# minghanz/bev

Hardware: NVIDIA B200
Metric: BEV warp Mpix/s (higher is better)
Workload: dtype u8

## Files before the change

bev_b200/csrc/warp_fast.cu:

```cuda
#include "bevk_common.cuh"
#include "warp_u8c3.cuh"
#include "warp_f16c3.cuh"
#include "warp_formats.cuh"

#include <cuda.h>
#include <mutex>
#include <string.h>

namespace {

template <typename PX, bool LINEAR> constexpr int cta_threads()
{
    return LINEAR ? PX::kLinearThreads : PX::kNearestThreads;
}
__host__ __device__ constexpr int tile_w(int segs) { return 32 * segs; }
__host__ __device__ constexpr int tile_h(int segs, int warps) { return warps * (4 / segs); }
constexpr int kNarrowW = 12, kNarrowH = 16, kWideW = 4, kWideH = 8;
constexpr int kMapCount = kNarrowW * kNarrowH + kWideW * kWideH;
constexpr int kMaxBoxWidth = 2048, kMaxBoxHeight = 32;
constexpr int kMaxBoxes = 3;
constexpr int kMaxStageFrames = 8;
constexpr int kBarBytes = 256;
constexpr int kPrefetchAhead = 2;
constexpr int kTailSlack = 64;

__host__ __device__ constexpr int map_width(int wi)
{
    return wi < 8 ? 64 * (wi + 1) : (wi < 12 ? 512 + 128 * (wi - 7) : 1024 + 256 * (wi - 11));
}
__host__ __device__ constexpr bool map_is_wide(int wi) { return wi >= kNarrowW; }
__host__ __device__ constexpr int map_height(int hi)
{
    return hi < 8 ? hi + 1 : (hi < 12 ? 10 + 2 * (hi - 8) : 20 + 4 * (hi - 12));
}
__host__ __device__ __forceinline__ int map_width_index(int bytes)
{
    return bytes <= 512 ? (bytes + 63) / 64 - 1
                        : (bytes <= 1024 ? 7 + (bytes - 512 + 127) / 128 : 11 + (bytes - 1024 + 255) / 256);
}
__host__ __device__ __forceinline__ int map_height_index(int rows)
{
    return rows <= 8 ? rows - 1 : (rows <= 16 ? 8 + (rows - 9) / 2 : 12 + (rows - 17) / 4);
}
__host__ __device__ __forceinline__ int box_height(int wi, int rows)
{
    return map_is_wide(wi) ? (rows + 3) / 4 * 4 : map_height(map_height_index(rows));
}
__host__ __device__ __forceinline__ int box_map_index(int wi, int rows)
{
    return map_is_wide(wi) ? kNarrowW * kNarrowH + (wi - kNarrowW) * kWideH + (rows + 3) / 4 - 1
                           : wi * kNarrowH + map_height_index(rows);
}

struct WarpFastMaps {
    CUtensorMap m[kMapCount];
};

constexpr int kMaxChunks = 12;
struct ChunkPlan {
    int n_chunks;
    uint32_t cum[kMaxChunks + 1];
};

constexpr int kRecWords = 8;
constexpr int kHdrInts = 8;
struct WarpScratch {
    int *next_item;
    int *ready;
    int *hdr;
    uint32_t *rec;
    uint32_t recip_per_chunk, recip_tiles, recip_tiles_y;
};

__device__ __forceinline__ uint32_t smem_u32(const void *p)
{
    return (uint32_t)__cvta_generic_to_shared(p);
}
__device__ __forceinline__ void mbar_init(uint32_t bar, uint32_t count)
{
    asm volatile("mbarrier.init.shared::cta.b64 [%0], %1;" ::"r"(bar), "r"(count));
}
__device__ __forceinline__ void mbar_expect_tx(uint32_t bar, uint32_t bytes)
{
    asm volatile("mbarrier.arrive.expect_tx.shared::cta.b64 _, [%0], %1;" ::"r"(bar), "r"(bytes)
                 : "memory");
}
__device__ __forceinline__ void mbar_arrive(uint32_t bar)
{
    asm volatile("mbarrier.arrive.shared::cta.b64 _, [%0];" ::"r"(bar) : "memory");
}
__device__ __forceinline__ void mbar_wait(uint32_t bar, uint32_t parity)
{
    asm volatile(
        "{\n\t"
        ".reg .pred p;\n\t"
        "WAIT_%=:\n\t"
        "mbarrier.try_wait.parity.shared::cta.b64 p, [%0], %1;\n\t"
        "@p bra DONE_%=;\n\t"
        "bra WAIT_%=;\n\t"
        "DONE_%=:\n\t"
        "}" ::"r"(bar),
        "r"(parity)
        : "memory");
}
__device__ __forceinline__ void tma_box_g2s(uint32_t dst, const CUtensorMap *map, int x, int y,
                                            uint32_t bar)
{
    asm volatile(
        "cp.async.bulk.tensor.2d.shared::cluster.global.mbarrier::complete_tx::bytes"
        " [%0], [%1, {%3, %4}], [%2];" ::"r"(dst),
        "l"(reinterpret_cast<uint64_t>(map)), "r"(bar), "r"(x), "r"(y)
        : "memory");
}
__device__ __forceinline__ void tma_box_prefetch(const CUtensorMap *map, int x, int y)
{
    asm volatile("cp.async.bulk.prefetch.tensor.2d.L2.global [%0, {%1, %2}];" ::"l"(
                     reinterpret_cast<uint64_t>(map)),
                 "r"(x), "r"(y)
                 : "memory");
}
__device__ __forceinline__ uint32_t lds32(uint32_t addr)
{
    uint32_t v;
    asm volatile("ld.shared.u32 %0, [%1];" : "=r"(v) : "r"(addr));
    return v;
}
__device__ __forceinline__ int ld_acquire(const int *p)
{
    int v;
    asm volatile("ld.acquire.gpu.global.s32 %0, [%1];" : "=r"(v) : "l"(p) : "memory");
    return v;
}
__device__ __forceinline__ void st_release(int *p, int v)
{
    asm volatile("st.release.gpu.global.s32 [%0], %1;" ::"l"(p), "r"(v) : "memory");
}
__device__ __forceinline__ void keep(uint32_t &v) { asm volatile("" : "+r"(v)); }
__device__ __forceinline__ void keep(int &v) { asm volatile("" : "+r"(v)); }

struct BoxPlan {
    int n_boxes;
    int x;
    int y0;
    uint32_t bytes;
    int frame0, frame_step;
    int src_h;
    int n_frames, fps;
    int slog;
    uint32_t ring, full0;
    uint32_t stride, frame_bytes, pitch;
    int map_idx[kMaxBoxes];
    int row[kMaxBoxes];
};

struct ItemDesc {
    int item;
    int gi, tile_x, tile_y;
    int f0, n_frames;
    int first, stride;
    int chunk;
    int ready;
};

struct LoopCtx {
    uint32_t ring, full0;
    uint32_t stride;
    uint32_t frame_bytes;
    uint32_t pitch;
    int fps;
    int n_frames;
    int slog;
    int ahead;
    const WarpFastMaps *maps;
    const BoxPlan *plan;
};

template <bool TO_SMEM>
__device__ __noinline__ void produce(const BoxPlan *plan, const WarpFastMaps *maps, int i0,
                                     uint32_t use, int lane)
{
    const BoxPlan &pl = *plan;
    const int nf = min(pl.fps, pl.n_frames - i0);
    const int nb = pl.n_boxes;
    const int f = nb == 1 ? lane : (nb == 2 ? lane >> 1 : (lane * 11) >> 5);
    const int b = lane - f * nb;
    const bool mine = f < nf;
    const int row = pl.row[mine ? b : 0];
    const CUtensorMap *map = &maps->m[pl.map_idx[mine ? b : 0]];
    const int y = (pl.frame0 + (i0 + f) * pl.frame_step) * pl.src_h + pl.y0 + row;
    if (TO_SMEM) {
        const uint32_t slot = use & ((1u << pl.slog) - 1u);
        const uint32_t fb = pl.full0 + 8 * slot;
        mbar_wait(fb + (8u << pl.slog), ((use >> pl.slog) & 1u) ^ 1u);
        if (lane == 0) mbar_expect_tx(fb, pl.bytes * nf);
        __syncwarp();
        if (mine)
            tma_box_g2s(pl.ring + slot * pl.stride + f * pl.frame_bytes + row * pl.pitch, map, pl.x, y, fb);
    } else if (mine) {
        tma_box_prefetch(map, pl.x, y);
    }
}

template <int WARPS>
__device__ __forceinline__ void feed(const LoopCtx &c, int done, uint32_t use, int lane, int warp)
{
    const int turn = ((int)use - warp) & (WARPS - 1);
    const int i_load = done + (c.ahead - 1) * c.fps;
    if (turn == 0 && i_load < c.n_frames) produce<true>(c.plan, c.maps, i_load, use + c.ahead, lane);
    if (c.slog == 1 && turn == WARPS / 2 && i_load + kPrefetchAhead * c.fps < c.n_frames)
        produce<false>(c.plan, c.maps, i_load + kPrefetchAhead * c.fps, 0, lane);
}

template <int WARPS, typename BODY, typename STARTED>
__device__ __forceinline__ uint32_t stage_loop(const LoopCtx &c, uint32_t use, uint8_t *d,
                                               const uint32_t d_step, const int tid, BODY body, STARTED started)
{
    const uint32_t smask = (1u << c.slog) - 1u;
    const int lane = tid & 31, warp = tid >> 5;
    if (warp == 0) {
        for (int s = 0; s < c.ahead && s * c.fps < c.n_frames; ++s)
            produce<true>(c.plan, c.maps, s * c.fps, use + s, lane);
        for (int s = c.ahead; c.slog == 1 && s < c.ahead + kPrefetchAhead && s * c.fps < c.n_frames; ++s)
            produce<false>(c.plan, c.maps, s * c.fps, 0, lane);
        if (tid == 0) started();
    }
    int done = 0;
#pragma unroll 1
    while (done < c.n_frames) {
        const uint32_t slot = use & smask;
        const uint32_t fb = c.full0 + 8 * slot;
        mbar_wait(fb, (use >> c.slog) & 1u);
        uint32_t sa = c.ring + slot * c.stride;
        int nf = min(c.fps, c.n_frames - done);
        done += nf;
#pragma unroll 1
        for (; nf > 0; --nf, sa += c.frame_bytes, d += d_step) body(sa, d);
        __syncwarp();
        if (lane == 0) mbar_arrive(fb + (8u << c.slog));
        feed<WARPS>(c, done, use, lane, warp);
        ++use;
    }
    return use;
}

template <int SEGS, bool PAIRS> __device__ __forceinline__ int warp_px_x(int warp)
{
    if (!PAIRS) return 0;
    return SEGS >= 2 ? 64 * (warp % (SEGS >= 2 ? SEGS / 2 : 1)) : 0;
}
template <int SEGS, bool PAIRS> __device__ __forceinline__ int warp_px_y(int warp)
{
    if (!PAIRS) return warp * (4 / SEGS);
    return SEGS >= 2 ? 2 * (warp / (SEGS >= 2 ? SEGS / 2 : 1)) : 4 * warp;
}
template <int SEGS, bool PAIRS> __device__ __forceinline__ constexpr int px_seg(int k)
{
    return PAIRS ? (SEGS >= 2 ? (k >> 1) : 0) : k % SEGS;
}
template <int SEGS, bool PAIRS> __device__ __forceinline__ constexpr int px_row(int k)
{
    return PAIRS ? (SEGS >= 2 ? (k & 1) : k) : k / SEGS;
}

struct PairReg {
    uint32_t addr;
    uint32_t sh;
    uint32_t sel_f, sel_s;
    uint32_t sel_y;
    uint32_t wf0, wf1;
    uint32_t ws0, ws1;
};

// ... 22 lines not shown
{
    const uint32_t rnd = 32768u;
    {
        const uint32_t x0 = prmt(a0.g0, a0.g1, q.sel_f), x1 = prmt(a1.g0, a1.g1, q.sel_f);
        const uint32_t t0 = __dp2a_lo(q.wf1, x1, __dp2a_lo(q.wf0, x0, rnd));
        const uint32_t t1 = __dp2a_hi(q.wf1, x1, __dp2a_hi(q.wf0, x0, rnd));
        const uint32_t t2 = __dp2a_lo(q.wf1, ya1, __dp2a_lo(q.wf0, ya0, rnd));
        pf = prmt(prmt(t0, t1, 0x4462u), t2, 0x7610u);
    }
    {
        const uint32_t x0 = prmt(b0.g0, b0.g1, q.sel_s), x1 = prmt(b1.g0, b1.g1, q.sel_s);
        const uint32_t t0 = __dp2a_lo(q.ws1, x1, __dp2a_lo(q.ws0, x0, rnd));
        const uint32_t t1 = __dp2a_hi(q.ws1, x1, __dp2a_hi(q.ws0, x0, rnd));
        const uint32_t t2 = __dp2a_hi(q.ws1, yb1, __dp2a_hi(q.ws0, yb0, rnd));
        ps = prmt(prmt(t0, t1, 0x4462u), t2, 0x7610u);
    }
}

template <typename PX, bool LINEAR, int MINB, int SEGS>
__global__ void __launch_bounds__((cta_threads<PX, LINEAR>()), MINB)
warp_fast_kernel(const __grid_constant__ BevkWarpParams p,
                      const __grid_constant__ WarpFastMaps maps,
                      const __grid_constant__ ChunkPlan plan, const int tiles_x, const int tiles_y,
                      const int total_items, const int ring_bytes, const WarpScratch sc)
{
    constexpr int kThreads = cta_threads<PX, LINEAR>(), kWarps = kThreads / 32;
    extern __shared__ __align__(128) uint8_t smem[];
    uint64_t *bars = reinterpret_cast<uint64_t *>(smem + ring_bytes);
    __shared__ int s_box[4];
    __shared__ int s_any;
    __shared__ uint32_t s_use[3];
    __shared__ ItemDesc s_item[2];
    __shared__ double s_M[BEVK_MAX_GROUPS][9];
    __shared__ BoxPlan s_plan;

    const int tid = threadIdx.x, lane = tid & 31, warp = tid >> 5;
    const uint32_t ring = smem_u32(smem);
    const uint32_t bar0 = smem_u32(bars);
    if (tid == 0) {
        for (int sl = 1; sl <= 3; ++sl) {
            const int S = 1 << sl, base = 16 * S - 32;
            for (int i = 0; i < S; ++i) {
                mbar_init(bar0 + base + 8 * i, 1);
                mbar_init(bar0 + base + 8 * (S + i), kWarps);
            }
            s_use[sl - 1] = 0;
        }
        asm volatile("fence.mbarrier_init.release.cluster;" ::: "memory");
    }

    const int n_tiles = tiles_x * tiles_y;
    const uint8_t *src = (const uint8_t *)p.src;
    uint8_t *dst = (uint8_t *)p.dst;
    constexpr int kBpp = PX::kBpp;
    constexpr bool kPairMap = LINEAR && PX::kPairs;
    const int src_row_bytes = p.src_w * kBpp;
    const long long src_frame_bytes = (long long)src_row_bytes * p.src_h;
    const long long dst_frame_bytes = (long long)p.dst_w * p.dst_h * kBpp;

    const int per_chunk = p.n_groups * n_tiles;
    auto fast_div = [](int n, int d, uint32_t recip) {
        uint32_t q = __umulhi((uint32_t)n, recip);
        if (q * (uint32_t)d > (uint32_t)n) --q;
        if ((q + 1u) * (uint32_t)d <= (uint32_t)n) ++q;
        return (int)q;
    };
    auto decode = [&](int item, ItemDesc &o) {
        o.item = item;
        if (item >= total_items) return;
        const int chunk = fast_div(item, per_chunk, sc.recip_per_chunk), rem = item - chunk * per_chunk;
        const int gi = fast_div(rem, n_tiles, sc.recip_tiles), tile = rem - gi * n_tiles;
        o.gi = gi;
        o.tile_x = fast_div(tile, tiles_y, sc.recip_tiles_y);
        o.tile_y = tile - o.tile_x * tiles_y;
        const int count = p.g[gi].count;
        o.f0 = (int)(((unsigned long long)count * plan.cum[chunk]) >> 16);
        o.n_frames = (int)(((unsigned long long)count * plan.cum[chunk + 1]) >> 16) - o.f0;
        o.first = p.g[gi].first;
        o.stride = p.g[gi].stride;
        o.chunk = chunk;
        o.ready = (sc.ready != nullptr && chunk > 0)
                      ? ld_acquire(sc.ready + (gi * n_tiles + o.tile_x * tiles_y + o.tile_y))
                      : 1;
    };
    for (int i = tid; i < p.n_groups * 9; i += kThreads) s_M[i / 9][i % 9] = p.g[i / 9].M[i % 9];
    if (tid == 0) {
        decode(atomicAdd(sc.next_item, 1), s_item[0]);
        s_box[0] = s_box[2] = 1 << 30;
        s_box[1] = s_box[3] = -1;
        s_any = 0;
    }
    __syncthreads();
    const bool bw0_pow2 = (p.bw0 & (p.bw0 - 1)) == 0;
    const uint32_t row_bytes = (uint32_t)p.dst_w * (uint32_t)kBpp;

    int par = 0;
#pragma unroll 1
    while (true) {
        const int item = s_item[par].item;
        if (item >= total_items) break;
        const int gi = s_item[par].gi, tile_x = s_item[par].tile_x, tile_y = s_item[par].tile_y;
        const int f0 = s_item[par].f0, n_frames = s_item[par].n_frames;
        const int g_first = s_item[par].first, g_stride = s_item[par].stride;
        const int chunk = s_item[par].chunk;
        const bool published = s_item[par].ready != 0;
        int next_raw = 0;
        if (tid == 0) next_raw = atomicAdd(sc.next_item, 1);
        const int x0 = tile_x * tile_w(SEGS) + warp_px_x<SEGS, kPairMap>(warp);
        const int y0 = tile_y * tile_h(SEGS, kWarps) + warp_px_y<SEGS, kPairMap>(warp);
        const int tile_id = gi * n_tiles + tile_x * tiles_y + tile_y;
        par ^= 1;

        int cs[4], rs[4];
        uint32_t wpk[4];
        int bx0, bx1, by0, by1;
        bool any;
        if (sc.ready == nullptr || chunk == 0) {
            bx0 = by0 = 1 << 30;
            bx1 = by1 = -1;
#pragma unroll
            for (int k = 0; k < 4; ++k) {
                const int x = x0 + lane + 32 * px_seg<SEGS, kPairMap>(k), y = y0 + px_row<SEGS, kPairMap>(k);
                const bool in_dst = (x < p.dst_w) && (y < p.dst_h);
                int X, Y, wc0, wc1, wr0, wr1;
                const int xc = min(x, p.dst_w - 1);
                const int xb = bw0_pow2 ? (xc & ~(p.bw0 - 1)) : (xc / p.bw0) * p.bw0;
                bevk_map_pixel_xb(s_M[gi], xb, xc - xb, min(y, p.dst_h - 1), LINEAR ? 32.0 : 1.0, X, Y);
                if (LINEAR) {
                    const int sx = bevk_sat16(X >> 5), sy = bevk_sat16(Y >> 5);
// ... 44 lines not shown
                    int4 *h = reinterpret_cast<int4 *>(sc.hdr + (size_t)tile_id * kHdrInts);
                    __stcg(h, make_int4(bx0, bx1, by0, by1));
                    __stcg(h + 1, make_int4(any ? 1 : 0, 0, 0, 0));
                }
                __threadfence();
            }
        } else {
            if (!published) {
                if (tid == 0) {
                    const int *flag = sc.ready + tile_id;
                    while (ld_acquire(flag) == 0) __nanosleep(100);
                }
            }
            __syncthreads();
            const int4 *h = reinterpret_cast<const int4 *>(sc.hdr + (size_t)tile_id * kHdrInts);
            const int4 hb = __ldcg(h), hf = __ldcg(h + 1);
            bx0 = hb.x;
            bx1 = hb.y;
            by0 = hb.z;
            by1 = hb.w;
            any = hf.x != 0;
            const uint32_t *rec = sc.rec + (size_t)tile_id * (kRecWords * kThreads) + tid;
#pragma unroll
            for (int k = 0; k < 4; ++k) {
                const uint32_t pos = __ldcg(rec + (2 * k) * kThreads);
                cs[k] = (int)(pos & 0xffffu);
                rs[k] = (int)(pos >> 16);
                wpk[k] = __ldcg(rec + (2 * k + 1) * kThreads);
            }
        }

        const int a0 = (kBpp * bx0) & ~15;
        const int need_w = ((kBpp * (bx1 + 1) + 15) & ~15) - a0;
        const int wi = map_width_index(need_w);
        const int pitch = map_width(wi);
        const int nrows = by1 - by0 + 1;
        bool staged = any && need_w <= kMaxBoxWidth && nrows <= kMaxBoxes * kMaxBoxHeight;
        int box_rows = 0;
        if (staged)
            for (int rem = nrows; rem > 0;) {
                const int h = box_height(wi, min(rem, kMaxBoxHeight));
                box_rows += h;
                rem -= h;
            }
        const uint32_t frame_bytes = ((uint32_t)(box_rows * pitch) + 127u) & ~127u;
        staged = staged && 2 * frame_bytes <= (uint32_t)ring_bytes;
        if (!LINEAR && frame_bytes > 3u * 1024u * (uint32_t)kBpp) staged = false;
        const int fps = 4 * kMaxStageFrames * frame_bytes <= (uint32_t)ring_bytes ? kMaxStageFrames
                        : 4 * 4 * frame_bytes <= (uint32_t)ring_bytes ? 4
                        : 8 * frame_bytes <= (uint32_t)ring_bytes ? 2 : 1;
        const int stage_stride = fps * (int)frame_bytes;
        const int slog = (8 * stage_stride <= ring_bytes) ? 3 : (4 * stage_stride <= ring_bytes ? 2 : 1);
        const uint32_t full0 = bar0 + 16 * (1 << slog) - 32;
        if (tid == 0) {
            if (staged) {
                int rem = nrows, row = 0, nb = 0;
                while (rem > 0) {
                    const int r = min(rem, kMaxBoxHeight);
                    s_plan.map_idx[nb] = box_map_index(wi, r);
                    s_plan.row[nb] = row;
                    row += box_height(wi, r);
                    rem -= box_height(wi, r);
                    ++nb;
                }
                s_plan.n_boxes = nb;
                s_plan.x = map_is_wide(wi) ? a0 >> 3 : a0 >> 2;
                s_plan.y0 = by0;
                s_plan.bytes = (uint32_t)(box_rows * pitch);
                s_plan.frame0 = g_first + f0 * g_stride;
                s_plan.frame_step = g_stride;
                s_plan.src_h = p.src_h;
                s_plan.n_frames = n_frames;
                s_plan.fps = fps;
                s_plan.slog = slog;
                s_plan.ring = ring;
                s_plan.full0 = full0;
                s_plan.stride = stage_stride;
                s_plan.frame_bytes = frame_bytes;
                s_plan.pitch = pitch;
            }
        }
        __syncthreads();
        if (tid == 0) {
            if (sc.ready != nullptr && chunk == 0) st_release(sc.ready + tile_id, 1);
            s_box[0] = s_box[2] = 1 << 30;
            s_box[1] = s_box[3] = -1;
            s_any = 0;
        }
        auto next_item_decode = [&]() { decode(next_raw, s_item[par]); };

        const typename PX::Store st = PX::store_setup(lane);
        bool seg_ok[4];
#pragma unroll
        for (int k = 0; k < 4; ++k) {
            const int valid_px = min(32, p.dst_w - (x0 + 32 * px_seg<SEGS, kPairMap>(k)));
            seg_ok[k] = (y0 + px_row<SEGS, kPairMap>(k) < p.dst_h) && PX::lane_stores(lane, valid_px);
        }
        auto seg_ptr = [row_bytes](uint8_t *dd, uint8_t *dd1, int k) -> uint8_t * {
            const int row = px_row<SEGS, kPairMap>(k), seg = px_seg<SEGS, kPairMap>(k);
            return (row & 1 ? dd1 : dd) + (row >> 1) * 2 * (size_t)row_bytes + PX::kSegBytes * seg;
        };
        uint32_t d_step = (uint32_t)g_stride * (uint32_t)dst_frame_bytes;
        keep(d_step);
        uint8_t *d = dst + (long long)(g_first + f0 * g_stride) * dst_frame_bytes +
                     ((long long)y0 * p.dst_w + x0) * kBpp + PX::lane_offset(lane);

        if ((!any || !staged) && tid == 0) next_item_decode();
        if (!any) {
#pragma unroll 1
            for (int i = 0; i < n_frames; ++i, d += d_step)
#pragma unroll
                for (int k = 0; k < 4; ++k) PX::store_zero(seg_ptr(d, d + row_bytes, k), seg_ok[k], lane);
        } else if (staged) {
            LoopCtx c;
            c.ring = ring;
            c.full0 = full0;
            c.stride = stage_stride;
            c.frame_bytes = frame_bytes;
            c.pitch = pitch;
            c.fps = fps;
            c.n_frames = n_frames;
            c.slog = slog;
            c.ahead = slog == 1 ? 2 : (1 << slog) - 1;
            c.maps = &maps;
            c.plan = &s_plan;
            keep(c.ring);
            keep(c.full0);
            keep(c.slog);
            uint32_t use = s_use[slog - 1];

            int var = 3;
            if constexpr (LINEAR && PX::kPairs) {
                bool ok0 = true, ok1 = true, ok2 = true;
#pragma unroll
                for (int j = 0; j < 2; ++j) {
                    const int a = 2 * j, b = a + 1;
                    const bool aa = wpk[a] != 0, ab = wpk[b] != 0;
                    if (aa && ab) {
                        const int dr = rs[b] - rs[a], dc = cs[b] - cs[a];
                        const bool near = dc >= -1 && dc <= 1;
                        ok0 = ok0 && near && dr == 0;
                        ok1 = ok1 && near && dr == 1;
                        ok2 = ok2 && near && dr == -1;
                    } else if (aa || ab) {
                        const int r = aa ? rs[a] : rs[b];
                        ok1 = ok1 && (aa ? r + 2 <= by1 : r - 1 >= by0);
                        ok2 = ok2 && (ab ? r + 2 <= by1 : r - 1 >= by0);
                    } else {
                        ok1 = ok1 && by1 - by0 >= 2;
                        ok2 = ok2 && by1 - by0 >= 2;
                    }
                }
                var = __all_sync(0xffffffffu, ok0) ? 0
                      : (__all_sync(0xffffffffu, ok1) ? 1 : (__all_sync(0xffffffffu, ok2) ? 2 : 3));
            }
            if constexpr (LINEAR && PX::kPairs) if (var != 3) {
                PairReg pr[2];
                uint32_t ok = 0;
// ... 142 lines not shown
    long long rows = 0;
    unsigned long long stamp = 0;
    WarpFastMaps maps;
};
constexpr int kMapCacheSize = 8;
MapCacheEntry g_map_cache[kMapCacheSize];
unsigned long long g_map_stamp = 0;
std::mutex g_map_mutex;
EncodeTiledFn g_encode = nullptr;

int get_maps(const void *base, int row_bytes, long long rows, WarpFastMaps &out)
{
    std::lock_guard<std::mutex> lock(g_map_mutex);
    if (!g_encode) {
        void *fn = nullptr;
        cudaDriverEntryPointQueryResult qres;
        BEVK_CUDA(cudaGetDriverEntryPoint("cuTensorMapEncodeTiled", &fn, cudaEnableDefault, &qres));
        if (qres != cudaDriverEntryPointSuccess || !fn)
            BEVK_FAIL(BEVK_E_CUDA, "cuTensorMapEncodeTiled is not available from this driver");
        g_encode = (EncodeTiledFn)fn;
    }
    MapCacheEntry *victim = &g_map_cache[0];
    for (int i = 0; i < kMapCacheSize; ++i) {
        MapCacheEntry &e = g_map_cache[i];
        if (e.base == base && e.row_bytes == row_bytes && e.rows == rows) {
            e.stamp = ++g_map_stamp;
            out = e.maps;
            return BEVK_OK;
        }
        if (e.stamp < victim->stamp) victim = &e;
    }
    const cuuint64_t gstride[1] = {(cuuint64_t)row_bytes};
    const cuuint32_t estride[2] = {1, 1};
    for (int wi = 0; wi < kNarrowW + kWideW; ++wi) {
        const bool wide = map_is_wide(wi);
        const int es = wide ? 8 : 4;
        const cuuint64_t gdim[2] = {(cuuint64_t)(row_bytes / es), (cuuint64_t)rows};
        for (int hi = 0; hi < (wide ? kWideH : kNarrowH); ++hi) {
            const int h = wide ? 4 * (hi + 1) : map_height(hi);
            const cuuint32_t box[2] = {(cuuint32_t)(map_width(wi) / es), (cuuint32_t)h};
            CUresult r = g_encode(&victim->maps.m[box_map_index(wi, h)],
                                  wide ? CU_TENSOR_MAP_DATA_TYPE_UINT64 : CU_TENSOR_MAP_DATA_TYPE_UINT32,
                                  2, const_cast<void *>(base), gdim, gstride, box, estride,
                                  CU_TENSOR_MAP_INTERLEAVE_NONE, CU_TENSOR_MAP_SWIZZLE_NONE,
                                  CU_TENSOR_MAP_L2_PROMOTION_L2_128B,
                                  CU_TENSOR_MAP_FLOAT_OOB_FILL_NONE);
            if (r != CUDA_SUCCESS) {
                victim->base = nullptr;
                BEVK_FAIL(BEVK_E_CUDA, "cuTensorMapEncodeTiled failed (code %d) for a %ux%u box",
                          (int)r, box[0] * es, box[1]);
            }
        }
    }
    victim->base = base;
    victim->row_bytes = row_bytes;
    victim->rows = rows;
    victim->stamp = ++g_map_stamp;
    out = victim->maps;
    return BEVK_OK;
}

struct KernelConfig {
    bool ready = false;
    int ctas_per_sm = 0;
    int ring_bytes = 0;
};
template <typename PX, bool LINEAR> constexpr int min_ctas()
{
    return LINEAR ? PX::kLinearCtas : 4 * (256 / cta_threads<PX, LINEAR>());
}
constexpr int kMaxDevices = 64;
struct DeviceState {
    KernelConfig cfg[5][2][3];
    int sm_count = 0;
    bool pool_ready = false;
};
DeviceState g_dev[kMaxDevices];
inline int segs_index(int segs) { return segs == 4 ? 0 : (segs == 2 ? 1 : 2); }

inline int format_index(int dtype, int channels)
{
    if (dtype == BEVK_U8) return channels == 3 ? 0 : (channels == 1 ? 2 : (channels == 4 ? 3 : -1));
    if (dtype == BEVK_F16) return channels == 3 ? 1 : -1;
    if (dtype == BEVK_F32) return channels == 3 ? 4 : -1;
// ... 88 lines not shown
        for (int iy = 0; iy < nsy; ++iy)
            for (int ix = 0; ix < nsx; ++ix) {
                const int ty = nsy > 1 ? (int)((long long)iy * (tiles_y - 1) / (nsy - 1)) : 0;
                const int tx = nsx > 1 ? (int)((long long)ix * (tiles_x - 1) / (nsx - 1)) : 0;
                const int x0 = tx * tw, y0 = ty * th;
                const int x1 = (x0 + tw < p.dst_w ? x0 + tw : p.dst_w) - 1;
                const int y1 = (y0 + th < p.dst_h ? y0 + th : p.dst_h) - 1;
                const int cx[4] = {x0, x1, x0, x1}, cy[4] = {y0, y0, y1, y1};
                int lo_x = 1 << 30, hi_x = -(1 << 30), lo_y = 1 << 30, hi_y = -(1 << 30), pos = 0, neg = 0;
                for (int c = 0; c < 4; ++c) {
                    const double w = M[6] * cx[c] + M[7] * cy[c] + M[8];
                    pos += w > 0;
                    neg += w < 0;
                    int X, Y;
                    bevk_map_pixel(M, cx[c], cy[c], p.bw0, scale, X, Y);
                    const int sx = bevk_sat16(linear ? (X >> 5) : X), sy = bevk_sat16(linear ? (Y >> 5) : Y);
                    lo_x = sx < lo_x ? sx : lo_x;
                    hi_x = sx > hi_x ? sx : hi_x;
                    lo_y = sy < lo_y ? sy : lo_y;
                    hi_y = sy > hi_y ? sy : hi_y;
                }
                hi_x += linear;
                hi_y += linear;
                if (hi_x < 0 || hi_y < 0 || lo_x >= p.src_w || lo_y >= p.src_h) continue;
                if (pos != 4 && neg != 4) continue;
                ++active;
                lo_x = lo_x < 0 ? 0 : lo_x;
                lo_y = lo_y < 0 ? 0 : lo_y;
                hi_x = hi_x > p.src_w - 1 ? p.src_w - 1 : hi_x;
                hi_y = hi_y > p.src_h - 1 ? p.src_h - 1 : hi_y;
                const int a0 = (bpp * lo_x) & ~15;
                const int need_w = ((bpp * (hi_x + 1) + 15) & ~15) - a0 + 16;
                const int rows = hi_y - lo_y + 1 + 1;
                const int pitch = need_w <= kMaxBoxWidth ? map_width(map_width_index(need_w)) : need_w;
                if (need_w > kMaxBoxWidth || rows > kMaxBoxes * kMaxBoxHeight ||
                    2LL * pitch * (rows + 3) > ring_bytes)
                    ++bad;
            }
    }
    return active ? (double)bad / (double)active : 0.0;
}

struct ModeKey {
    double M[BEVK_MAX_GROUPS][9];
    int n_groups, src_h, src_w, dst_h, dst_w, linear, bpp, warps;
};
struct ModeEntry {
    ModeKey key;
    int segs;
    int best;
    bool split;
    unsigned long long stamp = 0;
    bool valid = false;
};
constexpr double kMaxSplit = 0.35;
constexpr int kModeCacheSize = 8;
ModeEntry g_mode_cache[kModeCacheSize];
unsigned long long g_mode_stamp = 0;

int pick_tile_shape(const BevkWarpParams &p, int linear, int bpp, int warps, int ring_bytes, bool force, bool *split)
{
    const double kNegligible = linear ? 0.002 : 0.05;
    ModeKey key;
    memset(&key, 0, sizeof(key));
    for (int i = 0; i < p.n_groups; ++i) memcpy(key.M[i], p.g[i].M, sizeof(key.M[i]));
    key.n_groups = p.n_groups;
    key.src_h = p.src_h;
    key.src_w = p.src_w;
    key.dst_h = p.dst_h;
// ... 108 lines not shown
    if (rc) return rc;

    const int tiles_x = (p.dst_w + tile_w(segs) - 1) / tile_w(segs);
    const int tiles_y = (p.dst_h + tile_h(segs, warps) - 1) / tile_h(segs, warps);
    const long long n_tiles = (long long)tiles_x * tiles_y;
    const int ctas = ds.sm_count * cfg.ctas_per_sm;

    ChunkPlan plan;
    memset(&plan, 0, sizeof(plan));
    const long long tile_groups = n_tiles * p.n_groups;
    if (max_count >= 128 && tile_groups * 5 >= 2LL * ctas) {
        static const uint32_t cum[8] = {0, 20480, 36864, 49152, 57344, 61952, 64512, 65536};
        plan.n_chunks = 7;
        memcpy(plan.cum, cum, sizeof(cum));
    } else {
        int k = (int)((3LL * ctas + tile_groups - 1) / tile_groups);
        k = k < 1 ? 1 : k;
        k = k > kMaxChunks ? kMaxChunks : k;
        k = k > (max_count + 7) / 8 ? (max_count + 7) / 8 : k;
        k = k < 1 ? 1 : k;
        plan.n_chunks = k;
        for (int i = 0; i <= k; ++i) plan.cum[i] = (uint32_t)(65536LL * i / k);
    }
    const long long items = tile_groups * plan.n_chunks;
    if (items > 0x7fffffffLL) return 0;
    const int grid = (int)(items < ctas ? items : ctas);

    const bool share_setup = (fmt == 0 || fmt == 2) && linear && plan.n_chunks > 1 &&
                             tile_groups * kRecWords * threads * 4 <= (512LL << 20);
    const size_t off_hard = 256;
    const size_t off_ready = off_hard + (((size_t)(split ? tile_groups : 0) + 255) & ~(size_t)255);
    const size_t off_hdr = off_ready + (((size_t)(share_setup ? tile_groups * 4 : 0) + 255) & ~(size_t)255);
    const size_t off_rec = off_hdr + (share_setup ? (size_t)tile_groups * kHdrInts * 4 : 0);
    const size_t total = off_rec + (share_setup ? (size_t)tile_groups * kRecWords * threads * 4 : 0);
    unsigned char *scratch = nullptr;
    BEVK_CUDA(cudaMallocAsync((void **)&scratch, total, stream));
    cudaError_t e = cudaMemsetAsync(scratch, 0, off_hdr, stream);
    WarpScratch sc;
    sc.next_item = (int *)scratch;
    sc.ready = share_setup ? (int *)(scratch + off_ready) : nullptr;
    sc.hdr = share_setup ? (int *)(scratch + off_hdr) : nullptr;
    sc.rec = share_setup ? (uint32_t *)(scratch + off_rec) : nullptr;
    auto recip = [](long long d) { return d <= 1 ? 0xffffffffu : (uint32_t)(((1ULL << 32) + d - 1) / d); };
    sc.recip_per_chunk = recip(tile_groups);
    sc.recip_tiles = recip(n_tiles);
    sc.recip_tiles_y = recip(tiles_y);
    if (split) {
        p.hard = scratch + off_hard;
        p.hard_tw = tile_w(segs);
        p.hard_th = tile_h(segs, warps);
        p.hard_ty = tiles_y;
        p.hard_tiles = (int)n_tiles;
    }

    int rc2 = 0;
    if (e == cudaSuccess) {
        const int smem = cfg.ring_bytes + kBarBytes + kTailSlack;
        with_format(fmt, [&](auto px) {
            launch_any<decltype(px)>(linear, segs, grid, smem, stream, p, maps, plan, tiles_x, tiles_y, (int)items,
                                     cfg.ring_bytes, sc);
            return 0;
        });
        e = cudaGetLastError();
        if (e == cudaSuccess && split) {
            rc2 = bevk_plan_generic_chunks(p, channels);
            if (!rc2) rc2 = bevk_launch_warp_generic(p, channels, dtype, linear, stream);
        }
    }
    const cudaError_t ef = cudaFreeAsync(scratch, stream);
    if (e != cudaSuccess) {
        bevk_set_error("staged warp launch failed: %s", cudaGetErrorString(e));
        return BEVK_E_CUDA;
    }
    if (rc2) return rc2;
    BEVK_CUDA(ef);
// ... 3 lines not shown
```

Baseline: 686,700.

## Build per-item TMA descriptors on device with exact box dims

```diff
diff --git a/bev_b200/csrc/warp_fast.cu b/bev_b200/csrc/warp_fast.cu
--- a/bev_b200/csrc/warp_fast.cu
+++ b/bev_b200/csrc/warp_fast.cu
@@ -15,45 +15,14 @@
 }
 __host__ __device__ constexpr int tile_w(int segs) { return 32 * segs; }
 __host__ __device__ constexpr int tile_h(int segs, int warps) { return warps * (4 / segs); }
-constexpr int kNarrowW = 12, kNarrowH = 16, kWideW = 4, kWideH = 8;
-constexpr int kMapCount = kNarrowW * kNarrowH + kWideW * kWideH;
-constexpr int kMaxBoxWidth = 2048, kMaxBoxHeight = 32;
-constexpr int kMaxBoxes = 3;
+constexpr int kMaxNarrowWidth = 1024, kMaxBoxWidth = 2048, kMaxBoxRows = 256;
 constexpr int kMaxStageFrames = 8;
 constexpr int kBarBytes = 256;
 constexpr int kPrefetchAhead = 2;
 constexpr int kTailSlack = 64;
 
-__host__ __device__ constexpr int map_width(int wi)
-{
-    return wi < 8 ? 64 * (wi + 1) : (wi < 12 ? 512 + 128 * (wi - 7) : 1024 + 256 * (wi - 11));
-}
-__host__ __device__ constexpr bool map_is_wide(int wi) { return wi >= kNarrowW; }
-__host__ __device__ constexpr int map_height(int hi)
-{
-    return hi < 8 ? hi + 1 : (hi < 12 ? 10 + 2 * (hi - 8) : 20 + 4 * (hi - 12));
-}
-__host__ __device__ __forceinline__ int map_width_index(int bytes)
-{
-    return bytes <= 512 ? (bytes + 63) / 64 - 1
-                        : (bytes <= 1024 ? 7 + (bytes - 512 + 127) / 128 : 11 + (bytes - 1024 + 255) / 256);
-}
-__host__ __device__ __forceinline__ int map_height_index(int rows)
-{
-    return rows <= 8 ? rows - 1 : (rows <= 16 ? 8 + (rows - 9) / 2 : 12 + (rows - 17) / 4);
-}
-__host__ __device__ __forceinline__ int box_height(int wi, int rows)
-{
-    return map_is_wide(wi) ? (rows + 3) / 4 * 4 : map_height(map_height_index(rows));
-}
-__host__ __device__ __forceinline__ int box_map_index(int wi, int rows)
-{
-    return map_is_wide(wi) ? kNarrowW * kNarrowH + (wi - kNarrowW) * kWideH + (rows + 3) / 4 - 1
-                           : wi * kNarrowH + map_height_index(rows);
-}
-
 struct WarpFastMaps {
-    CUtensorMap m[kMapCount];
+    CUtensorMap m[2];
 };
 
 constexpr int kMaxChunks = 12;
@@ -69,6 +38,7 @@
     int *ready;
     int *hdr;
     uint32_t *rec;
+    CUtensorMap *tmaps;
     uint32_t recip_per_chunk, recip_tiles, recip_tiles_y;
 };
 
@@ -119,6 +89,24 @@
                  "r"(x), "r"(y)
                  : "memory");
 }
+__device__ __forceinline__ void tmap_set_box_dim(uint32_t smap, int dim, int v)
+{
+    if (dim == 0)
+        asm volatile("tensormap.replace.tile.box_dim.shared::cta.b1024.b32 [%0], 0, %1;" ::"r"(smap), "r"(v) : "memory");
+    else
+        asm volatile("tensormap.replace.tile.box_dim.shared::cta.b1024.b32 [%0], 1, %1;" ::"r"(smap), "r"(v) : "memory");
+}
+__device__ __forceinline__ void tmap_publish(CUtensorMap *gmap, uint32_t smap)
+{
+    asm volatile("tensormap.cp_fenceproxy.global.shared::cta.tensormap::generic.release.gpu.sync.aligned"
+                 " [%0], [%1], 128;" ::"l"(reinterpret_cast<uint64_t>(gmap)), "r"(smap)
+                 : "memory");
+}
+__device__ __forceinline__ void tmap_acquire(const CUtensorMap *gmap)
+{
+    asm volatile("fence.proxy.tensormap::generic.acquire.gpu [%0], 128;" ::"l"(reinterpret_cast<uint64_t>(gmap))
+                 : "memory");
+}
 __device__ __forceinline__ uint32_t lds32(uint32_t addr)
 {
     uint32_t v;
@@ -139,7 +127,7 @@
 __device__ __forceinline__ void keep(int &v) { asm volatile("" : "+r"(v)); }
 
 struct BoxPlan {
-    int n_boxes;
+    const CUtensorMap *map;
     int x;
     int y0;
     uint32_t bytes;
@@ -148,9 +136,7 @@
     int n_frames, fps;
     int slog;
     uint32_t ring, full0;
-    uint32_t stride, frame_bytes, pitch;
-    int map_idx[kMaxBoxes];
-    int row[kMaxBoxes];
+    uint32_t stride, frame_bytes;
 };
 
 struct ItemDesc {
@@ -171,23 +157,16 @@
     int n_frames;
     int slog;
     int ahead;
-    const WarpFastMaps *maps;
     const BoxPlan *plan;
 };
 
 template <bool TO_SMEM>
-__device__ __noinline__ void produce(const BoxPlan *plan, const WarpFastMaps *maps, int i0,
-                                     uint32_t use, int lane)
+__device__ __noinline__ void produce(const BoxPlan *plan, int i0, uint32_t use, int lane)
 {
     const BoxPlan &pl = *plan;
     const int nf = min(pl.fps, pl.n_frames - i0);
-    const int nb = pl.n_boxes;
-    const int f = nb == 1 ? lane : (nb == 2 ? lane >> 1 : (lane * 11) >> 5);
-    const int b = lane - f * nb;
-    const bool mine = f < nf;
-    const int row = pl.row[mine ? b : 0];
-    const CUtensorMap *map = &maps->m[pl.map_idx[mine ? b : 0]];
-    const int y = (pl.frame0 + (i0 + f) * pl.frame_step) * pl.src_h + pl.y0 + row;
+    const bool mine = lane < nf;
+    const int y = (pl.frame0 + (i0 + lane) * pl.frame_step) * pl.src_h + pl.y0;
     if (TO_SMEM) {
         const uint32_t slot = use & ((1u << pl.slog) - 1u);
         const uint32_t fb = pl.full0 + 8 * slot;
@@ -195,9 +174,9 @@
         if (lane == 0) mbar_expect_tx(fb, pl.bytes * nf);
         __syncwarp();
         if (mine)
-            tma_box_g2s(pl.ring + slot * pl.stride + f * pl.frame_bytes + row * pl.pitch, map, pl.x, y, fb);
+            tma_box_g2s(pl.ring + slot * pl.stride + lane * pl.frame_bytes, pl.map, pl.x, y, fb);
     } else if (mine) {
-        tma_box_prefetch(map, pl.x, y);
+        tma_box_prefetch(pl.map, pl.x, y);
     }
 }
 
@@ -206,9 +185,9 @@
 {
     const int turn = ((int)use - warp) & (WARPS - 1);
     const int i_load = done + (c.ahead - 1) * c.fps;
-    if (turn == 0 && i_load < c.n_frames) produce<true>(c.plan, c.maps, i_load, use + c.ahead, lane);
+    if (turn == 0 && i_load < c.n_frames) produce<true>(c.plan, i_load, use + c.ahead, lane);
     if (c.slog == 1 && turn == WARPS / 2 && i_load + kPrefetchAhead * c.fps < c.n_frames)
-        produce<false>(c.plan, c.maps, i_load + kPrefetchAhead * c.fps, 0, lane);
+        produce<false>(c.plan, i_load + kPrefetchAhead * c.fps, 0, lane);
 }
 
 template <int WARPS, typename BODY, typename STARTED>
@@ -219,9 +198,9 @@
     const int lane = tid & 31, warp = tid >> 5;
     if (warp == 0) {
         for (int s = 0; s < c.ahead && s * c.fps < c.n_frames; ++s)
-            produce<true>(c.plan, c.maps, s * c.fps, use + s, lane);
+            produce<true>(c.plan, s * c.fps, use + s, lane);
         for (int s = c.ahead; c.slog == 1 && s < c.ahead + kPrefetchAhead && s * c.fps < c.n_frames; ++s)
-            produce<false>(c.plan, c.maps, s * c.fps, 0, lane);
+            produce<false>(c.plan, s * c.fps, 0, lane);
         if (tid == 0) started();
     }
     int done = 0;
@@ -327,6 +306,7 @@
     __shared__ ItemDesc s_item[2];
     __shared__ double s_M[BEVK_MAX_GROUPS][9];
     __shared__ BoxPlan s_plan;
+    __shared__ __align__(128) CUtensorMap s_tmap;
 
     const int tid = threadIdx.x, lane = tid & 31, warp = tid >> 5;
     const uint32_t ring = smem_u32(smem);
@@ -389,6 +369,7 @@
     const uint32_t row_bytes = (uint32_t)p.dst_w * (uint32_t)kBpp;
 
     int par = 0;
+    uint32_t n_staged = 0;
 #pragma unroll 1
     while (true) {
         const int item = s_item[par].item;
@@ -499,19 +480,10 @@
 
         const int a0 = (kBpp * bx0) & ~15;
         const int need_w = ((kBpp * (bx1 + 1) + 15) & ~15) - a0;
-        const int wi = map_width_index(need_w);
-        const int pitch = map_width(wi);
+        const int pitch = need_w;
         const int nrows = by1 - by0 + 1;
-        bool staged = any && need_w <= kMaxBoxWidth && nrows <= kMaxBoxes * kMaxBoxHeight;
-        int box_rows = 0;
-        if (staged)
-            for (int rem = nrows; rem > 0;) {
-                const int h = box_height(wi, min(rem, kMaxBoxHeight));
-                box_rows += h;
-                rem -= h;
-            }
-        const uint32_t frame_bytes = ((uint32_t)(box_rows * pitch) + 127u) & ~127u;
-        staged = staged && 2 * frame_bytes <= (uint32_t)ring_bytes;
+        const uint32_t frame_bytes = ((uint32_t)nrows * (uint32_t)pitch + 127u) & ~127u;
+        bool staged = any && need_w <= kMaxBoxWidth && nrows <= kMaxBoxRows && 2 * frame_bytes <= (uint32_t)ring_bytes;
         if (!LINEAR && frame_bytes > 3u * 1024u * (uint32_t)kBpp) staged = false;
         const int fps = 4 * kMaxStageFrames * frame_bytes <= (uint32_t)ring_bytes ? kMaxStageFrames
                         : 4 * 4 * frame_bytes <= (uint32_t)ring_bytes ? 4
@@ -519,21 +491,26 @@
         const int stage_stride = fps * (int)frame_bytes;
         const int slog = (8 * stage_stride <= ring_bytes) ? 3 : (4 * stage_stride <= ring_bytes ? 2 : 1);
         const uint32_t full0 = bar0 + 16 * (1 << slog) - 32;
+        const bool wide = need_w > kMaxNarrowWidth;
+        CUtensorMap *tmap = sc.tmaps + 2 * blockIdx.x + (n_staged & 1u);
+        if (staged && warp == 0) {
+            const uint4 *base = reinterpret_cast<const uint4 *>(&maps.m[wide ? 1 : 0]);
+            if (lane < 8) reinterpret_cast<uint4 *>(&s_tmap)[lane] = base[lane];
+            __syncwarp();
+            const uint32_t smap = smem_u32(&s_tmap);
+            if (lane == 0) {
+                tmap_set_box_dim(smap, 0, need_w >> (wide ? 3 : 2));
+                tmap_set_box_dim(smap, 1, nrows);
+            }
+            __syncwarp();
+            tmap_publish(tmap, smap);
+        }
         if (tid == 0) {
             if (staged) {
-                int rem = nrows, row = 0, nb = 0;
-                while (rem > 0) {
-                    const int r = min(rem, kMaxBoxHeight);
-                    s_plan.map_idx[nb] = box_map_index(wi, r);
-                    s_plan.row[nb] = row;
-                    row += box_height(wi, r);
-                    rem -= box_height(wi, r);
-                    ++nb;
-                }
-                s_plan.n_boxes = nb;
-                s_plan.x = map_is_wide(wi) ? a0 >> 3 : a0 >> 2;
+                s_plan.map = tmap;
+                s_plan.x = wide ? a0 >> 3 : a0 >> 2;
                 s_plan.y0 = by0;
-                s_plan.bytes = (uint32_t)(box_rows * pitch);
+                s_plan.bytes = (uint32_t)nrows * (uint32_t)pitch;
                 s_plan.frame0 = g_first + f0 * g_stride;
                 s_plan.frame_step = g_stride;
                 s_plan.src_h = p.src_h;
@@ -544,10 +521,13 @@
                 s_plan.full0 = full0;
                 s_plan.stride = stage_stride;
                 s_plan.frame_bytes = frame_bytes;
-                s_plan.pitch = pitch;
             }
         }
         __syncthreads();
+        if (staged) {
+            tmap_acquire(tmap);
+            ++n_staged;
+        }
         if (tid == 0) {
             if (sc.ready != nullptr && chunk == 0) st_release(sc.ready + tile_id, 1);
             s_box[0] = s_box[2] = 1 << 30;
@@ -589,7 +569,6 @@
             c.n_frames = n_frames;
             c.slog = slog;
             c.ahead = slog == 1 ? 2 : (1 << slog) - 1;
-            c.maps = &maps;
             c.plan = &s_plan;
             keep(c.ring);
             keep(c.full0);
@@ -799,24 +778,18 @@
     }
     const cuuint64_t gstride[1] = {(cuuint64_t)row_bytes};
     const cuuint32_t estride[2] = {1, 1};
-    for (int wi = 0; wi < kNarrowW + kWideW; ++wi) {
-        const bool wide = map_is_wide(wi);
-        const int es = wide ? 8 : 4;
+    for (int i = 0; i < 2; ++i) {
+        const int es = i ? 8 : 4;
         const cuuint64_t gdim[2] = {(cuuint64_t)(row_bytes / es), (cuuint64_t)rows};
-        for (int hi = 0; hi < (wide ? kWideH : kNarrowH); ++hi) {
-            const int h = wide ? 4 * (hi + 1) : map_height(hi);
-            const cuuint32_t box[2] = {(cuuint32_t)(map_width(wi) / es), (cuuint32_t)h};
-            CUresult r = g_encode(&victim->maps.m[box_map_index(wi, h)],
-                                  wide ? CU_TENSOR_MAP_DATA_TYPE_UINT64 : CU_TENSOR_MAP_DATA_TYPE_UINT32,
-                                  2, const_cast<void *>(base), gdim, gstride, box, estride,
-                                  CU_TENSOR_MAP_INTERLEAVE_NONE, CU_TENSOR_MAP_SWIZZLE_NONE,
-                                  CU_TENSOR_MAP_L2_PROMOTION_L2_128B,
-                                  CU_TENSOR_MAP_FLOAT_OOB_FILL_NONE);
-            if (r != CUDA_SUCCESS) {
-                victim->base = nullptr;
-                BEVK_FAIL(BEVK_E_CUDA, "cuTensorMapEncodeTiled failed (code %d) for a %ux%u box",
-                          (int)r, box[0] * es, box[1]);
-            }
+        const cuuint32_t box[2] = {(cuuint32_t)(64 / es), 1};
+        CUresult r = g_encode(&victim->maps.m[i], i ? CU_TENSOR_MAP_DATA_TYPE_UINT64 : CU_TENSOR_MAP_DATA_TYPE_UINT32,
+                              2, const_cast<void *>(base), gdim, gstride, box, estride,
+                              CU_TENSOR_MAP_INTERLEAVE_NONE, CU_TENSOR_MAP_SWIZZLE_NONE,
+                              CU_TENSOR_MAP_L2_PROMOTION_L2_128B, CU_TENSOR_MAP_FLOAT_OOB_FILL_NONE);
+        if (r != CUDA_SUCCESS) {
+            victim->base = nullptr;
+            BEVK_FAIL(BEVK_E_CUDA, "cuTensorMapEncodeTiled failed (code %d) for the %d-byte element map",
+                      (int)r, es);
         }
     }
     victim->base = base;
@@ -971,9 +944,8 @@
                 const int a0 = (bpp * lo_x) & ~15;
                 const int need_w = ((bpp * (hi_x + 1) + 15) & ~15) - a0 + 16;
                 const int rows = hi_y - lo_y + 1 + 1;
-                const int pitch = need_w <= kMaxBoxWidth ? map_width(map_width_index(need_w)) : need_w;
-                if (need_w > kMaxBoxWidth || rows > kMaxBoxes * kMaxBoxHeight ||
-                    2LL * pitch * (rows + 3) > ring_bytes)
+                const long long frame_bytes = ((long long)need_w * rows + 127) & ~127LL;
+                if (need_w > kMaxBoxWidth || rows > kMaxBoxRows || 2 * frame_bytes > ring_bytes)
                     ++bad;
             }
     }
@@ -1148,7 +1120,8 @@
     const size_t off_ready = off_hard + (((size_t)(split ? tile_groups : 0) + 255) & ~(size_t)255);
     const size_t off_hdr = off_ready + (((size_t)(share_setup ? tile_groups * 4 : 0) + 255) & ~(size_t)255);
     const size_t off_rec = off_hdr + (share_setup ? (size_t)tile_groups * kHdrInts * 4 : 0);
-    const size_t total = off_rec + (share_setup ? (size_t)tile_groups * kRecWords * threads * 4 : 0);
+    const size_t off_tmaps = (off_rec + (share_setup ? (size_t)tile_groups * kRecWords * threads * 4 : 0) + 127) & ~(size_t)127;
+    const size_t total = off_tmaps + (size_t)grid * 2 * sizeof(CUtensorMap);
     unsigned char *scratch = nullptr;
     BEVK_CUDA(cudaMallocAsync((void **)&scratch, total, stream));
     cudaError_t e = cudaMemsetAsync(scratch, 0, off_hdr, stream);
@@ -1157,6 +1130,7 @@
     sc.ready = share_setup ? (int *)(scratch + off_ready) : nullptr;
     sc.hdr = share_setup ? (int *)(scratch + off_hdr) : nullptr;
     sc.rec = share_setup ? (uint32_t *)(scratch + off_rec) : nullptr;
+    sc.tmaps = (CUtensorMap *)(scratch + off_tmaps);
     auto recip = [](long long d) { return d <= 1 ? 0xffffffffu : (uint32_t)(((1ULL << 32) + d - 1) / d); };
     sc.recip_per_chunk = recip(tile_groups);
     sc.recip_tiles = recip(n_tiles);
```

Result: no change. 690,600, median of 6 (+0.6%).

## Precompute per-lane TMA copy requests in shared memory and interleave barrier pairs

Applied to the files above, without the earlier changes.

```diff
diff --git a/bev_b200/csrc/warp_fast.cu b/bev_b200/csrc/warp_fast.cu
--- a/bev_b200/csrc/warp_fast.cu
+++ b/bev_b200/csrc/warp_fast.cu
@@ -3,6 +3,7 @@
 #include "warp_f16c3.cuh"
 #include "warp_formats.cuh"
 
+#include <climits>
 #include <cuda.h>
 #include <mutex>
 #include <string.h>
@@ -125,6 +126,14 @@
     asm volatile("ld.shared.u32 %0, [%1];" : "=r"(v) : "r"(addr));
     return v;
 }
+__device__ __forceinline__ uint4 lds128(uint32_t addr)
+{
+    uint4 v;
+    asm volatile("ld.shared.v4.u32 {%0, %1, %2, %3}, [%4];"
+                 : "=r"(v.x), "=r"(v.y), "=r"(v.z), "=r"(v.w)
+                 : "r"(addr));
+    return v;
+}
 __device__ __forceinline__ int ld_acquire(const int *p)
 {
     int v;
@@ -138,20 +147,20 @@
 __device__ __forceinline__ void keep(uint32_t &v) { asm volatile("" : "+r"(v)); }
 __device__ __forceinline__ void keep(int &v) { asm volatile("" : "+r"(v)); }
 
-struct BoxPlan {
-    int n_boxes;
+struct CopyReq {
+    uint32_t off;
+    uint32_t map;
+    uint32_t y;
+    int f;
+};
+struct StagePlan {
     int x;
-    int y0;
+    uint32_t ystep;
     uint32_t bytes;
-    int frame0, frame_step;
-    int src_h;
-    int n_frames, fps;
-    int slog;
-    uint32_t ring, full0;
-    uint32_t stride, frame_bytes, pitch;
-    int map_idx[kMaxBoxes];
-    int row[kMaxBoxes];
-};
+    int n_frames;
+    CopyReq req[32];
+};
+__shared__ __align__(16) StagePlan s_plan;
 
 struct ItemDesc {
     int item;
@@ -172,72 +181,67 @@
     int slog;
     int ahead;
     const WarpFastMaps *maps;
-    const BoxPlan *plan;
 };
 
 template <bool TO_SMEM>
-__device__ __noinline__ void produce(const BoxPlan *plan, const WarpFastMaps *maps, int i0,
-                                     uint32_t use, int lane)
-{
-    const BoxPlan &pl = *plan;
-    const int nf = min(pl.fps, pl.n_frames - i0);
-    const int nb = pl.n_boxes;
-    const int f = nb == 1 ? lane : (nb == 2 ? lane >> 1 : (lane * 11) >> 5);
-    const int b = lane - f * nb;
-    const bool mine = f < nf;
-    const int row = pl.row[mine ? b : 0];
-    const CUtensorMap *map = &maps->m[pl.map_idx[mine ? b : 0]];
-    const int y = (pl.frame0 + (i0 + f) * pl.frame_step) * pl.src_h + pl.y0 + row;
+__device__ __noinline__ void produce(const WarpFastMaps *maps, int i0, int fps, uint32_t fb, uint32_t sa,
+                                     uint32_t parity)
+{
+    const int lane = threadIdx.x & 31;
+    const uint32_t plan = smem_u32(&s_plan);
+    const uint4 h = lds128(plan);
+    const uint4 r = lds128(plan + 16 + 16 * lane);
+    const int left = (int)h.w - i0;
+    const CUtensorMap *map = reinterpret_cast<const CUtensorMap *>(reinterpret_cast<const char *>(maps) + r.y);
+    const int y = (int)(r.z + (uint32_t)i0 * h.y);
     if (TO_SMEM) {
-        const uint32_t slot = use & ((1u << pl.slog) - 1u);
-        const uint32_t fb = pl.full0 + 8 * slot;
-        mbar_wait(fb + (8u << pl.slog), ((use >> pl.slog) & 1u) ^ 1u);
-        if (lane == 0) mbar_expect_tx(fb, pl.bytes * nf);
+        mbar_wait(fb + 8, parity);
+        if (lane == 0) mbar_expect_tx(fb, h.z * (uint32_t)min(fps, left));
         __syncwarp();
-        if (mine)
-            tma_box_g2s(pl.ring + slot * pl.stride + f * pl.frame_bytes + row * pl.pitch, map, pl.x, y, fb);
-    } else if (mine) {
-        tma_box_prefetch(map, pl.x, y);
-    }
-}
-
-template <int WARPS>
-__device__ __forceinline__ void feed(const LoopCtx &c, int done, uint32_t use, int lane, int warp)
-{
-    const int turn = ((int)use - warp) & (WARPS - 1);
-    const int i_load = done + (c.ahead - 1) * c.fps;
-    if (turn == 0 && i_load < c.n_frames) produce<true>(c.plan, c.maps, i_load, use + c.ahead, lane);
-    if (c.slog == 1 && turn == WARPS / 2 && i_load + kPrefetchAhead * c.fps < c.n_frames)
-        produce<false>(c.plan, c.maps, i_load + kPrefetchAhead * c.fps, 0, lane);
+        if ((int)r.w < left) tma_box_g2s(sa + r.x, map, (int)h.x, y, fb);
+    } else if ((int)r.w < left) {
+        tma_box_prefetch(map, (int)h.x, y);
+    }
 }
 
 template <int WARPS, typename BODY, typename STARTED>
 __device__ __forceinline__ uint32_t stage_loop(const LoopCtx &c, uint32_t use, uint8_t *d,
                                                const uint32_t d_step, const int tid, BODY body, STARTED started)
 {
-    const uint32_t smask = (1u << c.slog) - 1u;
+    const uint32_t last = (1u << c.slog) - 1u;
     const int lane = tid & 31, warp = tid >> 5;
     if (warp == 0) {
-        for (int s = 0; s < c.ahead && s * c.fps < c.n_frames; ++s)
-            produce<true>(c.plan, c.maps, s * c.fps, use + s, lane);
+        for (int s = 0; s < c.ahead && s * c.fps < c.n_frames; ++s) {
+            const uint32_t u = use + s, sl = u & last;
+            produce<true>(c.maps, s * c.fps, c.fps, c.full0 + 16 * sl, c.ring + sl * c.stride,
+                          ((u >> c.slog) & 1u) ^ 1u);
+        }
         for (int s = c.ahead; c.slog == 1 && s < c.ahead + kPrefetchAhead && s * c.fps < c.n_frames; ++s)
-            produce<false>(c.plan, c.maps, s * c.fps, 0, lane);
+            produce<false>(c.maps, s * c.fps, c.fps, 0, 0, 0);
         if (tid == 0) started();
     }
+    int i_load = c.ahead * c.fps;
     int done = 0;
 #pragma unroll 1
     while (done < c.n_frames) {
-        const uint32_t slot = use & smask;
-        const uint32_t fb = c.full0 + 8 * slot;
-        mbar_wait(fb, (use >> c.slog) & 1u);
+        const uint32_t slot = use & last, ph = (use >> c.slog) & 1u;
+        const uint32_t fb = c.full0 + 16 * slot;
+        mbar_wait(fb, ph);
         uint32_t sa = c.ring + slot * c.stride;
         int nf = min(c.fps, c.n_frames - done);
         done += nf;
 #pragma unroll 1
         for (; nf > 0; --nf, sa += c.frame_bytes, d += d_step) body(sa, d);
         __syncwarp();
-        if (lane == 0) mbar_arrive(fb + (8u << c.slog));
-        feed<WARPS>(c, done, use, lane, warp);
+        if (lane == 0) mbar_arrive(fb + 8);
+        const int turn = ((int)use - warp) & (WARPS - 1);
+        if (turn == 0 && i_load < c.n_frames) {
+            const uint32_t u = c.slog == 1 ? use : use - 1u, ts = u & last;
+            produce<true>(c.maps, i_load, c.fps, c.full0 + 16 * ts, c.ring + ts * c.stride, (u >> c.slog) & 1u);
+        }
+        if (c.slog == 1 && turn == WARPS / 2 && i_load + kPrefetchAhead * c.fps < c.n_frames)
+            produce<false>(c.maps, i_load + kPrefetchAhead * c.fps, c.fps, 0, 0, 0);
+        i_load += c.fps;
         ++use;
     }
     return use;
@@ -326,7 +330,6 @@
     __shared__ uint32_t s_use[3];
     __shared__ ItemDesc s_item[2];
     __shared__ double s_M[BEVK_MAX_GROUPS][9];
-    __shared__ BoxPlan s_plan;
 
     const int tid = threadIdx.x, lane = tid & 31, warp = tid >> 5;
     const uint32_t ring = smem_u32(smem);
@@ -335,8 +338,8 @@
         for (int sl = 1; sl <= 3; ++sl) {
             const int S = 1 << sl, base = 16 * S - 32;
             for (int i = 0; i < S; ++i) {
-                mbar_init(bar0 + base + 8 * i, 1);
-                mbar_init(bar0 + base + 8 * (S + i), kWarps);
+                mbar_init(bar0 + base + 16 * i, 1);
+                mbar_init(bar0 + base + 16 * i + 8, kWarps);
             }
             s_use[sl - 1] = 0;
         }
@@ -515,36 +518,25 @@
         if (!LINEAR && frame_bytes > 3u * 1024u * (uint32_t)kBpp) staged = false;
         const int fps = 4 * kMaxStageFrames * frame_bytes <= (uint32_t)ring_bytes ? kMaxStageFrames
                         : 4 * 4 * frame_bytes <= (uint32_t)ring_bytes ? 4
-                        : 8 * frame_bytes <= (uint32_t)ring_bytes ? 2 : 1;
+                        : 4 * frame_bytes <= (uint32_t)ring_bytes ? 2 : 1;
         const int stage_stride = fps * (int)frame_bytes;
         const int slog = (8 * stage_stride <= ring_bytes) ? 3 : (4 * stage_stride <= ring_bytes ? 2 : 1);
         const uint32_t full0 = bar0 + 16 * (1 << slog) - 32;
-        if (tid == 0) {
-            if (staged) {
-                int rem = nrows, row = 0, nb = 0;
-                while (rem > 0) {
-                    const int r = min(rem, kMaxBoxHeight);
-                    s_plan.map_idx[nb] = box_map_index(wi, r);
-                    s_plan.row[nb] = row;
-                    row += box_height(wi, r);
-                    rem -= box_height(wi, r);
-                    ++nb;
-                }
-                s_plan.n_boxes = nb;
+        if (warp == 0 && staged) {
+            const int nb = (nrows + kMaxBoxHeight - 1) / kMaxBoxHeight;
+            const int f = nb == 1 ? lane : (nb == 2 ? lane >> 1 : (lane * 11) >> 5);
+            const int row = (lane - f * nb) * kMaxBoxHeight;
+            const uint32_t y = ((uint32_t)g_first + (uint32_t)(f0 + f) * (uint32_t)g_stride) * (uint32_t)p.src_h +
+                               (uint32_t)(by0 + row);
+            *reinterpret_cast<uint4 *>(&s_plan.req[lane]) =
+                make_uint4((uint32_t)f * frame_bytes + (uint32_t)(row * pitch),
+                           (uint32_t)(box_map_index(wi, min(nrows - row, kMaxBoxHeight)) * sizeof(CUtensorMap)), y,
+                           f < fps ? f : INT_MAX);
+            if (lane == 0) {
                 s_plan.x = map_is_wide(wi) ? a0 >> 3 : a0 >> 2;
-                s_plan.y0 = by0;
+                s_plan.ystep = (uint32_t)g_stride * (uint32_t)p.src_h;
                 s_plan.bytes = (uint32_t)(box_rows * pitch);
-                s_plan.frame0 = g_first + f0 * g_stride;
-                s_plan.frame_step = g_stride;
-                s_plan.src_h = p.src_h;
                 s_plan.n_frames = n_frames;
-                s_plan.fps = fps;
-                s_plan.slog = slog;
-                s_plan.ring = ring;
-                s_plan.full0 = full0;
-                s_plan.stride = stage_stride;
-                s_plan.frame_bytes = frame_bytes;
-                s_plan.pitch = pitch;
             }
         }
         __syncthreads();
@@ -590,7 +582,6 @@
             c.slog = slog;
             c.ahead = slog == 1 ? 2 : (1 << slog) - 1;
             c.maps = &maps;
-            c.plan = &s_plan;
             keep(c.ring);
             keep(c.full0);
             keep(c.slog);
```

New measurement: 688,500 before, 711,500 after, median of 6. +3.3%, better.
